# robflynnyh/long-context-asr

Measured on AMD Instinct MI355X. Metric: spectrogram-frames/sec (6L/768D, seq=16384), higher is better.
Workload: dtype bf16; 1 GPU; 6L/768D/6H SConformerXL, seq=16384, rotary theta=1.5M, fwd+CTC+bwd+clip+MADGRAD; per_gpu_batch=128, global_batch=128, seq_len=16384, parallelism=dp1

## Files before the change

### long-context-asr_amd/csrc/attention.hip

```cpp
#ifdef SCONF_ATTN_STAMP
#define SCONF_STAMPS
#endif
#include "common.h"
#include <algorithm>
#include <type_traits>
#include <vector>
#include <stdio.h>

namespace {

struct AttnParams {
    const bf16 *q, *k, *v;
    bf16* o;
    const bf16 *dout;
    bf16 *dq, *dk, *dv;
    float* lse;
    float* delta;
    long q_sb, q_sn, q_sh, k_sb, k_sn, k_sh, v_sb, v_sn, v_sh, o_sb, o_sn, o_sh;
    long do_sb, do_sn, do_sh, dq_sb, dq_sn, dq_sh, dk_sb, dk_sn, dk_sh, dv_sb, dv_sn, dv_sh;
    const int* lengths;
    int B, N, H;
    int win_left, win_right;
    float scale;
    const float *rot_cos, *rot_sin;
    unsigned long long* stamps;
};

#ifdef SCONF_ATTN_STAMP
#define STAMP_OUT(n) do { if (p.stamps && (threadIdx.x & 63) == 0) for (int i_ = 0; i_ < (n); ++i_) p.stamps[((long)blockIdx.x * 8 + (threadIdx.x >> 6)) * 8 + i_] = st_acc_[i_]; } while (0)
#else
#define STAMP_OUT(n)
#endif

struct BlkId { int b, h, x; };
__device__ __forceinline__ BlkId decode_block(const AttnParams& p, int nx) {
    const int total = nx * p.H * p.B, v = blockIdx.x;
    const int q = total >> 3, r = total & 7, xcd = v & 7;
    const int lid = (xcd < r ? xcd * (q + 1) : r * (q + 1) + (xcd - r) * q) + (v >> 3);
    BlkId o;
    o.x = lid % nx;
    const int bh = lid / nx;
    o.h = bh % p.H; o.b = bh / p.H;
    return o;
}

constexpr float RESCALE_LOG2 = 6.f;

template <int D> __device__ __forceinline__ int swz(int row) {
    if constexpr (D == 32) return (row >> 2) & 3;
    else if constexpr (D == 64) return (((row >> 1) & 1) << 2) | (((row >> 3) & 1) << 1) | ((row >> 2) & 1);
    else return ((row & 3) << 2) | ((row >> 2) & 3);
}
template <int D> __device__ __forceinline__ int tile_off(int row, int ch) {
    return row * (2 * D) + ((ch ^ swz<D>(row)) << 4);
// ... 42 lines not shown
}

template <int D> struct LaneOffs {
    int row[D / 16];
    int trlo[D / 32];
    __device__ __forceinline__ LaneOffs(int lane) {
#pragma unroll
        for (int st = 0; st < D / 16; ++st) row[st] = tile_off<D>(lane & 31, 2 * st + (lane >> 5));
        const int i = lane & 15, q4 = i >> 2, p4 = i & 3, G = (lane >> 4) & 1, hh = lane >> 5;
        const int row0 = 4 * hh + q4, sub = (p4 & 1) * 8;
#pragma unroll
        for (int db = 0; db < D / 32; ++db) trlo[db] = tile_off<D>(row0, db * 4 + 2 * G + (p4 >> 1)) + sub;
    }
};
template <int D> __device__ __forceinline__ bf16x8 frag_row(const char* s, const LaneOffs<D>& L, int rbase, int st) {
    return *reinterpret_cast<const bf16x8*>(s + rbase * 2 * D + L.row[st]);
}
template <int D> __device__ __forceinline__ bf16x8 frag_tr(const char* s, const LaneOffs<D>& L, int rb, int db, int x32 = 32) {
    bf16x4 lo = __builtin_amdgcn_ds_read_tr16_b64_v4bf16((lds_p4)(s + rb * 2 * D + L.trlo[db]));
    bf16x4 hi = __builtin_amdgcn_ds_read_tr16_b64_v4bf16((lds_p4)(s + rb * 2 * D + 16 * D + (L.trlo[db] ^ x32)));
    return __builtin_shufflevector(lo, hi, 0, 1, 2, 3, 4, 5, 6, 7);
}
template <int D> __device__ __forceinline__ void load_bfrags(bf16x8 (&f)[D / 16], const bf16* base, long sn, int row0, int nvalid, int lane) {
    const int r = row0 + (lane & 31);
#pragma unroll
    for (int st = 0; st < D / 16; ++st) {
        uint4 v = make_uint4(0, 0, 0, 0);
        if (r < nvalid) v = *reinterpret_cast<const uint4*>(base + (long)r * sn + 16 * st + 8 * (lane >> 5));
        f[st] = __builtin_bit_cast(bf16x8, v);
    }
}
template <int D> __device__ __forceinline__ float delta_from_frags(const bf16x8 (&gf)[D / 16], const bf16* op, long o_sn, int row0, int nvalid, int lane) {
    bf16x8 of[D / 16];
    load_bfrags<D>(of, op, o_sn, row0, nvalid, lane);
    float acc = 0.f;
#pragma unroll
    for (int st = 0; st < D / 16; ++st)
#pragma unroll
        for (int j = 0; j < 8; ++j) acc += (float)gf[st][j] * (float)of[st][j];
    return acc + __shfl_xor(acc, 32, 64);
}
__device__ __forceinline__ bf16x8 pack8(const f32x16& a, int s2) {
    bf16x8 p;
#pragma unroll
    for (int j = 0; j < 8; ++j) p[j] = (bf16)a[8 * s2 + j];
    return p;
}

template <int D> __device__ __forceinline__ void store_t(const f32x16 (&acc)[D / 32], bf16* dst_row, float sc, int hh) {
#pragma unroll
    for (int db = 0; db < D / 32; ++db)
#pragma unroll
        for (int r4 = 0; r4 < 4; ++r4) {
            float v[4];
#pragma unroll
            for (int e = 0; e < 4; ++e) v[e] = acc[db][4 * r4 + e] * sc;
            store4(dst_row + db * 32 + 8 * r4 + 4 * hh, v);
        }
}

template <int D> __device__ __forceinline__ void store_t_rot(f32x16 (&acc)[D / 32], bf16* dst_row, float sc, int hh, const float* cs, const float* sn) {
    if constexpr (D >= 64) {
#pragma unroll
        for (int db = 0; db < D / 64; ++db)
#pragma unroll
            for (int r4 = 0; r4 < 4; ++r4) {
                float c[4], s[4];
                load4(cs + db * 32 + 8 * r4 + 4 * hh, c); load4(sn + db * 32 + 8 * r4 + 4 * hh, s);
#pragma unroll
                for (int e = 0; e < 4; ++e) {
                    const float a = acc[db][4 * r4 + e], b = acc[db + D / 64][4 * r4 + e];
                    acc[db][4 * r4 + e] = a * c[e] + b * s[e];
                    acc[db + D / 64][4 * r4 + e] = b * c[e] - a * s[e];
                }
            }
    } else {
#pragma unroll
        for (int r4 = 0; r4 < 2; ++r4) {
            float c[4], s[4];
            load4(cs + 8 * r4 + 4 * hh, c); load4(sn + 8 * r4 + 4 * hh, s);
#pragma unroll
            for (int e = 0; e < 4; ++e) {
                const float a = acc[0][4 * r4 + e], b = acc[0][4 * r4 + 8 + e];
                acc[0][4 * r4 + e] = a * c[e] + b * s[e];
                acc[0][4 * r4 + 8 + e] = b * c[e] - a * s[e];
            }
        }
    }
    store_t<D>(acc, dst_row, sc, hh);
}

template <int D>
__global__ __launch_bounds__(256, D == 256 ? 1 : 2) void attn_fwd_kernel(const AttnParams p) {
    extern __shared__ __attribute__((aligned(16))) char smem[];
    constexpr int TB = 64 * 2 * D;
    const int tid = threadIdx.x, lane = tid & 63, wave = tid >> 6, hh = lane >> 5;
    const BlkId bid = decode_block(p, (p.N + 127) / 128);
    const int b = bid.b, h = bid.h, qb0 = bid.x * 128, q0 = qb0 + wave * 32;
    const int len = p.lengths ? p.lengths[b] : p.N;
    const bf16* qp = p.q + b * p.q_sb + h * p.q_sh;
    const bf16* kp = p.k + b * p.k_sb + h * p.k_sh;
    const bf16* vp = p.v + b * p.v_sb + h * p.v_sh;
    const int qi = q0 + (lane & 31);
    const float c = p.scale * 1.4426950408889634f;

    bf16x8 qf[D / 16];
    load_bfrags<D>(qf, qp, p.q_sn, q0, p.N, lane);
    const LaneOffs<D> L(lane);

    const int kv_lo = p.win_left < 0 ? 0 : max(0, qb0 - p.win_left);
    const int kv_hi = min(len, p.win_right < 0 ? len : qb0 + 128 + p.win_right);
// ... 94 lines not shown
                                         float& d0, float& d1, float& d2, float& d3) {
    asm("v_fma_f32 %0, %8, %12, %13\n\tv_fma_f32 %1, %9, %12, %14\n\tv_fma_f32 %2, %10, %12, %15\n\tv_fma_f32 %3, %11, %12, %16\n\t"
        "v_exp_f32 %0, %0\n\tv_exp_f32 %1, %1\n\tv_exp_f32 %2, %2\n\tv_exp_f32 %3, %3\n\t"
        "v_mul_f32 %4, %4, %0\n\tv_mul_f32 %5, %5, %1\n\tv_mul_f32 %6, %6, %2\n\tv_mul_f32 %7, %7, %3"
        : "=&v"(pr[0]), "=&v"(pr[1]), "=&v"(pr[2]), "=&v"(pr[3]), "+v"(d0), "+v"(d1), "+v"(d2), "+v"(d3)
        : "v"(s0), "v"(s1), "v"(s2), "v"(s3), "v"(c), "v"(n0), "v"(n1), "v"(n2), "v"(n3));
}
__device__ __forceinline__ void exp4_submul(float s0, float s1, float s2, float s3, float c, float nl, float nd, float& d0, float& d1, float& d2, float& d3) {
    float e0, e1, e2, e3;
    asm("v_fma_f32 %0, %8, %12, %13\n\tv_fma_f32 %1, %9, %12, %13\n\tv_fma_f32 %2, %10, %12, %13\n\tv_fma_f32 %3, %11, %12, %13\n\t"
        "v_exp_f32 %0, %0\n\tv_exp_f32 %1, %1\n\tv_exp_f32 %2, %2\n\tv_exp_f32 %3, %3\n\t"
        "v_add_f32 %4, %4, %14\n\tv_add_f32 %5, %5, %14\n\tv_add_f32 %6, %6, %14\n\tv_add_f32 %7, %7, %14\n\t"
        "v_mul_f32 %4, %4, %0\n\tv_mul_f32 %5, %5, %1\n\tv_mul_f32 %6, %6, %2\n\tv_mul_f32 %7, %7, %3"
        : "=&v"(e0), "=&v"(e1), "=&v"(e2), "=&v"(e3), "+v"(d0), "+v"(d1), "+v"(d2), "+v"(d3)
        : "v"(s0), "v"(s1), "v"(s2), "v"(s3), "v"(c), "v"(nl), "v"(nd));
}
__device__ __forceinline__ void mfma_guard(f32x16& a) { asm volatile("s_nop 15\n\ts_nop 3" : "+v"(a)); }
__device__ __forceinline__ void mfma_guard(f32x16& a, f32x16& b) { asm volatile("s_nop 15\n\ts_nop 3" : "+v"(a), "+v"(b)); }

template <int D>
__global__ __launch_bounds__(512) void attn_fwd8p_kernel(const AttnParams p) {
    constexpr int KT = 128;
    extern __shared__ __attribute__((aligned(16))) char smem[];
    constexpr int TB = KT * 2 * D;
    const int tid = threadIdx.x, lane = tid & 63, wave = tid >> 6, hh = lane >> 5;
    const BlkId bid = decode_block(p, (p.N + 255) / 256);
    const int b = bid.b, h = bid.h, qb0 = bid.x * 256, q0 = qb0 + wave * 32;
    const int len = p.lengths ? p.lengths[b] : p.N;
    const bf16* qp = p.q + b * p.q_sb + h * p.q_sh;
    const bf16* kp = p.k + b * p.k_sb + h * p.k_sh;
    const bf16* vp = p.v + b * p.v_sb + h * p.v_sh;
    const int qi = q0 + (lane & 31);
    const float c = p.scale * 1.4426950408889634f;

    bf16x8 qf[D / 16];
    load_bfrags<D>(qf, qp, p.q_sn, q0, p.N, lane);
    const LaneOffs<D> L(lane);

    const int kv_lo = p.win_left < 0 ? 0 : max(0, qb0 - p.win_left);
    const int kv_hi = min(len, p.win_right < 0 ? len : qb0 + 256 + p.win_right);
    const int t_lo = kv_lo / KT, t_hi = (kv_hi + KT - 1) / KT;
    const bool windowed = p.win_left >= 0 || p.win_right >= 0;

    const unsigned lds0 = __builtin_amdgcn_readfirstlane(lds_addr(smem));
    const int wave_u = __builtin_amdgcn_readfirstlane(wave);
    const srd_t ksrd = make_srd(kp, view_bytes<D>(p.N, p.k_sn)), vsrd = make_srd(vp, view_bytes<D>(p.N, p.v_sn));
// ... 29 lines not shown

    f32x16 o[D / 32];
#pragma unroll
    for (int i = 0; i < D / 32; ++i)
#pragma unroll
        for (int r = 0; r < 16; ++r) o[i][r] = 0.f;
    float mc = 0.f, l0 = 0.f, l1 = 0.f;
    if (t_lo < t_hi) issue(t_lo, 0);
    pin_frags(qf);
    wait_vm<0>();
    __syncthreads();
    if (t_lo < t_hi) {
        const int kv0 = t_lo * KT;
        f32x16 s0, s1;
        s_chain(smem, 0, s0); s_chain(smem, 1, s1);
        if (kv0 + 64 > kv_hi || windowed) { mask_block(s0, kv0); mask_block(s1, kv0 + 32); }
        float mx = -INFINITY;
#pragma unroll
        for (int r = 0; r < 16; ++r) mx = fmaxf(mx, fmaxf(s0[r], s1[r]));
        mx = fmaxf(mx, __shfl_xor(mx, 32, 64));
        mc = (mx > -INFINITY) ? mx * c : 0.f;
    }
    const float nmc = -mc;
    STAMP_DECL(8)
    auto exp_block = [&](f32x16& sb, bf16x8& plo, bf16x8& phi) {
        mfma_guard(sb);
#pragma unroll
        for (int g = 0; g < 4; ++g) {
            float e[4];
            exp4_sum(e, sb[4 * g], sb[4 * g + 1], sb[4 * g + 2], sb[4 * g + 3], c, nmc, l0, l1);
#pragma unroll
            for (int j = 0; j < 4; ++j) sb[4 * g + j] = e[j];
        }
        plo = pack8(sb, 0); phi = pack8(sb, 1);
    };
    auto half_tile = [&](const char* sKh, const char* sVh, int kv0, const bool MASKED) {
        f32x16 s0, s1;
        bf16x8 pf[2][2];
        s_chain(sKh, 0, s0);
        if (MASKED) mask_block(s0, kv0);
        STAMP(1);
        s_chain(sKh, 1, s1);
        exp_block(s0, pf[0][0], pf[0][1]);
        if (MASKED) mask_block(s1, kv0 + 32);
        STAMP(2);
#pragma unroll
        for (int i = 0; i < 8; ++i)
// ... 2 lines not shown
        STAMP(3);
#pragma unroll
        for (int i = 0; i < 8; ++i)
            o[i >> 1] = __builtin_amdgcn_mfma_f32_32x32x16_bf16(frag_tr<D>(sVh, L, 32 + 16 * (i & 1), i >> 1), pf[1][i & 1], o[i >> 1], 0, 0, 0);
        STAMP(4);
    };
    for (int t = t_lo; t < t_hi; ++t) {
        const int cur = (t - t_lo) & 1;
        const char* sK = smem + cur * 2 * TB;
        const char* sV = sK + TB;
        if (t + 1 < t_hi) issue(t + 1, cur ^ 1);
        STAMP(0);
        for (int half = 0; half < KT / 64; ++half) {
            const int kv0 = t * KT + half * 64;
            if (kv0 >= kv_hi) break;
            const char* sKh = sK + half * 64 * 2 * D;
            const char* sVh = sV + half * 64 * 2 * D;
            half_tile(sKh, sVh, kv0, kv0 + 64 > kv_hi || windowed);
        }
        wait_vm<0>();
        __syncthreads();
        STAMP(5);
    }
    STAMP_OUT(6);
    float l = l0 + l1;
    float lt = l + __shfl_xor(l, 32, 64);
    float mfin = mc;
    if (__syncthreads_or(qi < len && qi < p.N && !(lt > 0.f && lt < 1e37f))) {
#pragma unroll
        for (int i = 0; i < D / 32; ++i)
#pragma unroll
            for (int r = 0; r < 16; ++r) o[i][r] = 0.f;
        float m = -INFINITY;
        l = 0.f;
        if (t_lo < t_hi) issue(t_lo, 0);
        wait_vm<0>();
        __syncthreads();
        for (int t = t_lo; t < t_hi; ++t) {
            const int cur = (t - t_lo) & 1;
            const char* sK = smem + cur * 2 * TB;
            const char* sV = sK + TB;
            if (t + 1 < t_hi) issue(t + 1, cur ^ 1);
            for (int half = 0; half < KT / 64; ++half) {
                const int kv0 = t * KT + half * 64;
                if (kv0 >= kv_hi) break;
                const char* sKh = sK + half * 64 * 2 * D;
                const char* sVh = sV + half * 64 * 2 * D;
// ... 23 lines not shown
                }
                l += rs;
                const bf16x8 p00 = pack8(s0, 0), p01 = pack8(s0, 1), p10 = pack8(s1, 0), p11 = pack8(s1, 1);
#pragma unroll
                for (int db = 0; db < D / 32; ++db) {
                    o[db] = __builtin_amdgcn_mfma_f32_32x32x16_bf16(frag_tr<D>(sVh, L, 0, db), p00, o[db], 0, 0, 0);
                    o[db] = __builtin_amdgcn_mfma_f32_32x32x16_bf16(frag_tr<D>(sVh, L, 16, db), p01, o[db], 0, 0, 0);
                    o[db] = __builtin_amdgcn_mfma_f32_32x32x16_bf16(frag_tr<D>(sVh, L, 32, db), p10, o[db], 0, 0, 0);
                    o[db] = __builtin_amdgcn_mfma_f32_32x32x16_bf16(frag_tr<D>(sVh, L, 48, db), p11, o[db], 0, 0, 0);
                }
            }
            wait_vm<0>();
            __syncthreads();
        }
        lt = l + __shfl_xor(l, 32, 64);
        mfin = (m == -INFINITY) ? 0.f : m * c;
    }
    if (qi < p.N) {
        const bool live = qi < len && lt > 0.f;
        const float inv = live ? 1.f / lt : 0.f;
        store_t<D>(o, p.o + b * p.o_sb + (long)qi * p.o_sn + h * p.o_sh, inv, hh);
        if (hh == 0 && p.lse) p.lse[((long)b * p.H + h) * p.N + qi] = live ? (mfin + __log2f(lt)) * 0.6931471805599453f : INFINITY;
    }
}

template <int D>
__global__ __launch_bounds__(256, D == 256 ? 1 : 2) void attn_bwd_dkdv_kernel(const AttnParams p) {
    extern __shared__ __attribute__((aligned(16))) char smem[];
    constexpr int TB = 32 * 2 * D;
    constexpr int SB = 2 * TB + 256;
    const int tid = threadIdx.x, lane = tid & 63, wave = tid >> 6, hh = lane >> 5;
    const BlkId bid = decode_block(p, (p.N + 127) / 128);
    const int b = bid.b, h = bid.h, kb0 = bid.x * 128, k0 = kb0 + wave * 32;
    const int len = p.lengths ? p.lengths[b] : p.N;
    const bf16* qp = p.q + b * p.q_sb + h * p.q_sh;
    const bf16* kp = p.k + b * p.k_sb + h * p.k_sh;
    const bf16* vp = p.v + b * p.v_sb + h * p.v_sh;
    const bf16* gp = p.dout + b * p.do_sb + h * p.do_sh;
    const float* delp = p.delta + ((long)b * p.H + h) * p.N;
    const float* lsep = delp + (long)p.B * p.H * p.N;
    const int key = k0 + (lane & 31);
    const float c = p.scale * 1.4426950408889634f;

    bf16x8 kf[D / 16];
    load_bfrags<D>(kf, kp, p.k_sn, k0, p.N, lane);
    const LaneOffs<D> L(lane);
// ... 78 lines not shown
            }
        }
        const bf16x8 pb0 = pack8(s, 0), pb1 = pack8(s, 1), db0 = pack8(dp, 0), db1 = pack8(dp, 1);
#pragma unroll
        for (int db = 0; db < D / 32; ++db) {
            dvt[db] = __builtin_amdgcn_mfma_f32_32x32x16_bf16(frag_tr<D>(sG, L, 0, db), pb0, dvt[db], 0, 0, 0);
            dvt[db] = __builtin_amdgcn_mfma_f32_32x32x16_bf16(frag_tr<D>(sG, L, 16, db), pb1, dvt[db], 0, 0, 0);
            dkt[db] = __builtin_amdgcn_mfma_f32_32x32x16_bf16(frag_tr<D>(sQ, L, 0, db), db0, dkt[db], 0, 0, 0);
            dkt[db] = __builtin_amdgcn_mfma_f32_32x32x16_bf16(frag_tr<D>(sQ, L, 16, db), db1, dkt[db], 0, 0, 0);
        }
        if (t + 1 < t_hi) lstore_stats(smem + (cur ^ 1) * SB);
        __syncthreads();
    }
    if (key < p.N) {
        if (p.rot_cos) store_t_rot<D>(dkt, p.dk + b * p.dk_sb + (long)key * p.dk_sn + h * p.dk_sh, p.scale, lane >> 5, p.rot_cos + (long)key * (D / 2), p.rot_sin + (long)key * (D / 2));
        else store_t<D>(dkt, p.dk + b * p.dk_sb + (long)key * p.dk_sn + h * p.dk_sh, p.scale, lane >> 5);
        store_t<D>(dvt, p.dv + b * p.dv_sb + (long)key * p.dv_sn + h * p.dv_sh, 1.f, lane >> 5);
    }
}

template <int D>
__global__ __launch_bounds__(512) void attn_bwd_dkdv8_kernel(const AttnParams p) {
    extern __shared__ __attribute__((aligned(16))) char smem[];
    constexpr int QR = 64;
    constexpr int TB = QR * 2 * D;
    constexpr int SB = 2 * TB + 512;
    const int tid = threadIdx.x, lane = tid & 63, wave = tid >> 6, hh = lane >> 5;
    const BlkId bid = decode_block(p, (p.N + 255) / 256);
    const int b = bid.b, h = bid.h, kb0 = bid.x * 256, k0 = kb0 + wave * 32;
    const int len = p.lengths ? p.lengths[b] : p.N;
    const bf16* qp = p.q + b * p.q_sb + h * p.q_sh;
    const bf16* kp = p.k + b * p.k_sb + h * p.k_sh;
    const bf16* vp = p.v + b * p.v_sb + h * p.v_sh;
    const bf16* gp = p.dout + b * p.do_sb + h * p.do_sh;
    const float* delp = p.delta + ((long)b * p.H + h) * p.N;
    const float* lsep = delp + (long)p.B * p.H * p.N;
    const int key = k0 + (lane & 31);
    const float c = p.scale * 1.4426950408889634f;

    bf16x8 kf[D / 16];
    load_bfrags<D>(kf, kp, p.k_sn, k0, p.N, lane);
    const LaneOffs<D> L(lane);
    char* sVt = smem + 2 * SB;
    const unsigned lds0 = __builtin_amdgcn_readfirstlane(lds_addr(smem));
    dma_tile<D, 256, 512>(vp, p.v_sn, kb0, p.N, lds0 + (unsigned)(2 * SB), tid);
    const char* sVw = sVt + wave * 32 * 2 * D;
// ... 9 lines not shown

    f32x16 dkt[D / 32], dvt[D / 32];
#pragma unroll
    for (int i = 0; i < D / 32; ++i)
#pragma unroll
        for (int r = 0; r < 16; ++r) { dkt[i][r] = 0.f; dvt[i][r] = 0.f; }

    const srd_t qsrd = make_srd(qp, view_bytes<D>(p.N, p.q_sn)), gsrd = make_srd(gp, view_bytes<D>(p.N, p.do_sn));
    auto issue = [&](int t, int buf) {
        const int tid_ = opaque(tid);
        const unsigned qvoff = tile_voff<D, 512>(p.q_sn, tid_), gvoff = tile_voff<D, 512>(p.do_sn, tid_);
        const int wave_u = __builtin_amdgcn_readfirstlane(tid_ >> 6);
        dma_tile128<QR, true>(qsrd, qvoff, p.q_sn, t * QR, lds0 + (unsigned)(buf * SB), wave_u);
        dma_tile128<QR, true>(gsrd, gvoff, p.do_sn, t * QR, lds0 + (unsigned)(buf * SB + TB), wave_u);
        if (wave_u < 2) {
            const int q = min(t * QR + (tid_ & 63), p.N - 1);
            dma4_asm((wave_u == 0 ? lsep : delp) + q, lds0 + (unsigned)(buf * SB + 2 * TB) + 256u * (unsigned)wave_u);
        }
    };
    if (t_lo < t_hi) issue(t_lo, 0);
    pin_frags(kf);
    wait_vm<0>();
    __syncthreads();
    STAMP_DECL(8)
    for (int t = t_lo; t < t_hi; ++t) {
        const int cur = (t - t_lo) & 1;
        const char* sQ = smem + cur * SB;
        const char* sG = sQ + TB;
        const float* sL = reinterpret_cast<const float*>(sQ + 2 * TB);
        const float* sD = sL + 64;
        if (t + 1 < t_hi) issue(t + 1, cur ^ 1);
        const bool need_mask = mask_wg || (t + 1) * QR > len;
        const int x32 = opaque(32);
        const int hh = (opaque(tid) >> 5) & 1;
        STAMP(0);
#pragma unroll
        for (int sub = 0; sub < 2; ++sub) {
            const int rb = 32 * sub, q0 = t * QR + rb;
            f32x16 s, dp;
#pragma unroll
            for (int g = 0; g < 4; ++g) {
                const float4 d4 = *reinterpret_cast<const float4*>(sD + rb + 8 * g + 4 * hh);
                dp[4 * g] = d4.x; dp[4 * g + 1] = d4.y; dp[4 * g + 2] = d4.z; dp[4 * g + 3] = d4.w;
            }
#pragma unroll
            for (int r = 0; r < 16; ++r) s[r] = 0.f;
#pragma unroll
// ... 15 lines not shown
                exp4_mul(pr, s[4 * g], s[4 * g + 1], s[4 * g + 2], s[4 * g + 3], c, a.x, a.y, a.z, a.w, d0, d1, d2, d3);
                dp[4 * g] = d0; dp[4 * g + 1] = d1; dp[4 * g + 2] = d2; dp[4 * g + 3] = d3;
#pragma unroll
                for (int e = 0; e < 4; ++e) s[4 * g + e] = pr[e];
            }
            bf16x8 pb0 = pack8(s, 0), pb1 = pack8(s, 1), db0 = pack8(dp, 0), db1 = pack8(dp, 1);
#ifdef SCONF_ATTN_STAMP
            tie(pb0); tie(pb1); tie(db0); tie(db1);
#endif
            STAMP(2);
#pragma unroll
            for (int db = 0; db < D / 32; ++db) {
                dvt[db] = __builtin_amdgcn_mfma_f32_32x32x16_bf16(frag_tr<D>(sG, L, rb, db, x32), pb0, dvt[db], 0, 0, 0);
                dvt[db] = __builtin_amdgcn_mfma_f32_32x32x16_bf16(frag_tr<D>(sG, L, rb + 16, db, x32), pb1, dvt[db], 0, 0, 0);
                dkt[db] = __builtin_amdgcn_mfma_f32_32x32x16_bf16(frag_tr<D>(sQ, L, rb, db, x32), db0, dkt[db], 0, 0, 0);
                dkt[db] = __builtin_amdgcn_mfma_f32_32x32x16_bf16(frag_tr<D>(sQ, L, rb + 16, db, x32), db1, dkt[db], 0, 0, 0);
            }
            STAMP(3);
        }
        wait_vm<0>();
        __syncthreads();
        STAMP(4);
    }
    STAMP_OUT(5);
    if (key < p.N) {
        if (p.rot_cos) store_t_rot<D>(dkt, p.dk + b * p.dk_sb + (long)key * p.dk_sn + h * p.dk_sh, p.scale, lane >> 5, p.rot_cos + (long)key * (D / 2), p.rot_sin + (long)key * (D / 2));
        else store_t<D>(dkt, p.dk + b * p.dk_sb + (long)key * p.dk_sn + h * p.dk_sh, p.scale, lane >> 5);
        store_t<D>(dvt, p.dv + b * p.dv_sb + (long)key * p.dv_sn + h * p.dv_sh, 1.f, lane >> 5);
    }
}

template <int D>
__global__ __launch_bounds__(256, D == 256 ? 1 : 2) void attn_bwd_dq_kernel(const AttnParams p) {
    extern __shared__ __attribute__((aligned(16))) char smem[];
    constexpr int TB = 64 * 2 * D;
    const int tid = threadIdx.x, lane = tid & 63, wave = tid >> 6, hh = lane >> 5;
    const BlkId bid = decode_block(p, (p.N + 127) / 128);
    const int b = bid.b, h = bid.h, qb0 = bid.x * 128, q0 = qb0 + wave * 32;
    const int len = p.lengths ? p.lengths[b] : p.N;
    const bf16* qp = p.q + b * p.q_sb + h * p.q_sh;
    const bf16* kp = p.k + b * p.k_sb + h * p.k_sh;
    const bf16* vp = p.v + b * p.v_sb + h * p.v_sh;
    const bf16* gp = p.dout + b * p.do_sb + h * p.do_sh;
    const int qi = q0 + (lane & 31);
    const float c = p.scale * 1.4426950408889634f;
    const float lse2 = (qi < len) ? p.lse[((long)b * p.H + h) * p.N + qi] * 1.4426950408889634f : INFINITY;

    bf16x8 qf[D / 16], gf[D / 16];
    load_bfrags<D>(qf, qp, p.q_sn, q0, p.N, lane);
    load_bfrags<D>(gf, gp, p.do_sn, q0, p.N, lane);
    float dlt = delta_from_frags<D>(gf, p.o + b * p.o_sb + h * p.o_sh, p.o_sn, q0, p.N, lane);
    if (qi >= len) dlt = 0.f;
// ... 48 lines not shown
                    if (p.win_right >= 0) ok = ok && key <= qi + p.win_right;
                    dp[r] = ok ? __builtin_amdgcn_exp2f(s[r] * c - lse2) * (dp[r] - dlt) : 0.f;
                }
            }
            const bf16x8 d0 = pack8(dp, 0), d1 = pack8(dp, 1);
#pragma unroll
            for (int db = 0; db < D / 32; ++db) {
                dqt[db] = __builtin_amdgcn_mfma_f32_32x32x16_bf16(frag_tr<D>(sK, L, kt * 32, db), d0, dqt[db], 0, 0, 0);
                dqt[db] = __builtin_amdgcn_mfma_f32_32x32x16_bf16(frag_tr<D>(sK, L, kt * 32 + 16, db), d1, dqt[db], 0, 0, 0);
            }
        }
        __syncthreads();
    }
    if (qi < p.N) {
        if (p.rot_cos) store_t_rot<D>(dqt, p.dq + b * p.dq_sb + (long)qi * p.dq_sn + h * p.dq_sh, p.scale, hh, p.rot_cos + (long)qi * (D / 2), p.rot_sin + (long)qi * (D / 2));
        else store_t<D>(dqt, p.dq + b * p.dq_sb + (long)qi * p.dq_sn + h * p.dq_sh, p.scale, hh);
    }
}

template <int D>
__global__ __launch_bounds__(512) void attn_bwd_dq8_kernel(const AttnParams p) {
    constexpr int KT = 128;
    extern __shared__ __attribute__((aligned(16))) char smem[];
    constexpr int TB = KT * 2 * D;
    const int tid = threadIdx.x, lane = tid & 63, wave = tid >> 6, hh = lane >> 5;
    const BlkId bid = decode_block(p, (p.N + 255) / 256);
    const int b = bid.b, h = bid.h, qb0 = bid.x * 256, q0 = qb0 + wave * 32;
    const int len = p.lengths ? p.lengths[b] : p.N;
    const bf16* qp = p.q + b * p.q_sb + h * p.q_sh;
    const bf16* kp = p.k + b * p.k_sb + h * p.k_sh;
    const bf16* vp = p.v + b * p.v_sb + h * p.v_sh;
    const bf16* gp = p.dout + b * p.do_sb + h * p.do_sh;
    const int qi = q0 + (lane & 31);
    const float c = p.scale * 1.4426950408889634f;
    const float lse2 = (qi < len) ? p.lse[((long)b * p.H + h) * p.N + qi] * 1.4426950408889634f : INFINITY;

    bf16x8 qf[D / 16], gf[D / 16];
    load_bfrags<D>(qf, qp, p.q_sn, q0, p.N, lane);
    load_bfrags<D>(gf, gp, p.do_sn, q0, p.N, lane);
    float dlt = delta_from_frags<D>(gf, p.o + b * p.o_sb + h * p.o_sh, p.o_sn, q0, p.N, lane);
    if (qi >= len) dlt = 0.f;
    if (hh == 0 && qi < p.N) {
        const long si = ((long)b * p.H + h) * p.N + qi;
        p.delta[si] = -dlt;
        p.delta[(long)p.B * p.H * p.N + si] = -lse2;
    }
    const LaneOffs<D> L(lane);
    const bool windowed = p.win_left >= 0 || p.win_right >= 0;
    const int key_lo = p.win_left >= 0 ? max(0, qi - p.win_left) : 0;
    const int key_hi = p.win_right >= 0 ? min(len - 1, qi + p.win_right) : len - 1;
    const unsigned key_rng = key_hi >= key_lo ? (unsigned)(key_hi - key_lo) : 0u;
    const bool key_none = key_hi < key_lo;

    const int kv_lo = p.win_left < 0 ? 0 : max(0, qb0 - p.win_left);
    const int kv_hi = min(len, p.win_right < 0 ? len : qb0 + 256 + p.win_right);
    const int t_lo = kv_lo / KT, t_hi = (qb0 < len) ? (kv_hi + KT - 1) / KT : t_lo;

    f32x16 dqt[D / 32];
#pragma unroll
    for (int i = 0; i < D / 32; ++i)
#pragma unroll
        for (int r = 0; r < 16; ++r) dqt[i][r] = 0.f;

    const unsigned lds0 = __builtin_amdgcn_readfirstlane(lds_addr(smem));
    const int wave_u = __builtin_amdgcn_readfirstlane(wave);
    const srd_t ksrd = make_srd(kp, view_bytes<D>(p.N, p.k_sn)), vsrd = make_srd(vp, view_bytes<D>(p.N, p.v_sn));
    const unsigned kvoff = tile_voff<D, 512>(p.k_sn, tid), vvoff = tile_voff<D, 512>(p.v_sn, tid);
    auto issue = [&](int t, int buf) {
        dma_tile128<KT, true>(ksrd, kvoff, p.k_sn, t * KT, lds0 + (unsigned)(buf * 2 * TB), wave_u);
        dma_tile128<KT, true>(vsrd, vvoff, p.v_sn, t * KT, lds0 + (unsigned)(buf * 2 * TB + TB), wave_u);
    };
    if (t_lo < t_hi) issue(t_lo, 0);
    pin_frags(qf); pin_frags(gf);
    wait_vm<0>();
    __syncthreads();
    STAMP_DECL(8)
    for (int t = t_lo; t < t_hi; ++t) {
        const int cur = (t - t_lo) & 1;
        const char* sK = smem + cur * 2 * TB;
        const char* sV = sK + TB;
        if (t + 1 < t_hi) issue(t + 1, cur ^ 1);
        STAMP(0);
        const int kv0 = t * KT;
        const bool masked = windowed || kv0 + KT > kv_hi;
        const float nl = -lse2, nd = -dlt;
        f32x16 s2[2], dp2[2];
        auto chains = [&](int kt, f32x16& s, f32x16& dp) {
#pragma unroll
            for (int r = 0; r < 16; ++r) { s[r] = 0.f; dp[r] = 0.f; }
#pragma unroll
            for (int st = 0; st < D / 16; ++st) {
                s = __builtin_amdgcn_mfma_f32_32x32x16_bf16(frag_row<D>(sK, L, kt * 32, st), qf[st], s, 0, 0, 0);
                dp = __builtin_amdgcn_mfma_f32_32x32x16_bf16(frag_row<D>(sV, L, kt * 32, st), gf[st], dp, 0, 0, 0);
            }
        };
        chains(0, s2[0], dp2[0]);
        STAMP(1);
#pragma unroll
        for (int kt = 0; kt < KT / 32; ++kt) {
// ... 8 lines not shown
            mfma_guard(s, dp);
#pragma unroll
            for (int g = 0; g < 4; ++g) {
                float d0 = dp[4 * g], d1 = dp[4 * g + 1], d2 = dp[4 * g + 2], d3 = dp[4 * g + 3];
                exp4_submul(s[4 * g], s[4 * g + 1], s[4 * g + 2], s[4 * g + 3], c, nl, nd, d0, d1, d2, d3);
                dp[4 * g] = d0; dp[4 * g + 1] = d1; dp[4 * g + 2] = d2; dp[4 * g + 3] = d3;
            }
            bf16x8 d0 = pack8(dp, 0), d1 = pack8(dp, 1);
#ifdef SCONF_ATTN_STAMP
            tie(d0); tie(d1);
#endif
            STAMP(2);
#pragma unroll
            for (int db = 0; db < D / 32; ++db) {
                dqt[db] = __builtin_amdgcn_mfma_f32_32x32x16_bf16(frag_tr<D>(sK, L, kt * 32, db), d0, dqt[db], 0, 0, 0);
                dqt[db] = __builtin_amdgcn_mfma_f32_32x32x16_bf16(frag_tr<D>(sK, L, kt * 32 + 16, db), d1, dqt[db], 0, 0, 0);
            }
            STAMP(3);
        }
        wait_vm<0>();
        __syncthreads();
        STAMP(4);
    }
    STAMP_OUT(5);
    if (qi < p.N) {
        if (p.rot_cos) store_t_rot<D>(dqt, p.dq + b * p.dq_sb + (long)qi * p.dq_sn + h * p.dq_sh, p.scale, hh, p.rot_cos + (long)qi * (D / 2), p.rot_sin + (long)qi * (D / 2));
        else store_t<D>(dqt, p.dq + b * p.dq_sb + (long)qi * p.dq_sn + h * p.dq_sh, p.scale, hh);
    }
}

#ifdef SCONF_ATTN_STAMP
static unsigned long long* stamp_buf(long nwg, hipStream_t stream) {
    static unsigned long long* sbuf = nullptr; static long scap = 0;
    if (scap < nwg * 64) { if (sbuf) (void)hipFree(sbuf); (void)hipMalloc(&sbuf, nwg * 64 * 8); scap = nwg * 64; }
    (void)hipMemsetAsync(sbuf, 0, nwg * 64 * 8, stream);
    return sbuf;
}
static void stamp_report(const char* what, unsigned long long* sbuf, long nwg, double units_per_wave, int nseg, const char* const* nm, hipStream_t stream) {
    if (!getenv("SCONF_ATTN_STAMP_PRINT")) return;
    (void)hipStreamSynchronize(stream);
    std::vector<unsigned long long> hb(nwg * 64);
    (void)hipMemcpy(hb.data(), sbuf, nwg * 64 * 8, hipMemcpyDeviceToHost);
    double sums[2][8] = {};
    for (long w = 0; w < nwg * 8; ++w) for (int i = 0; i < 8; ++i) sums[(w & 7) >= 4][i] += (double)hb[w * 8 + i];
    const double n = (double)nwg * 4 * units_per_wave;
    for (int g = 0; g < 2; ++g) {
        double tot = 0; for (int i = 0; i < nseg; ++i) tot += sums[g][i];
        fprintf(stderr, "[%s stamps] waves %d-%d: cycles per unit %.0f:", what, 4 * g, 4 * g + 3, tot / n);
        for (int i = 0; i < nseg; ++i) fprintf(stderr, "  %s %.0f (%.1f%%)", nm[i], sums[g][i] / n, 100.0 * sums[g][i] / tot);
        fprintf(stderr, "\n");
    }
// ... 52 lines not shown
SCONF_API int sconf_attn_fwd(const void* q, const void* k, const void* v, void* o, float* lse, const int32_t* lengths,
                             int64_t B, int64_t N, int64_t H, int64_t D, const int64_t* q_strides, const int64_t* k_strides,
                             const int64_t* v_strides, const int64_t* o_strides, int win_left, int win_right, float scale,
                             hipStream_t stream) {
    int64_t all[12];
    for (int i = 0; i < 3; ++i) { all[i] = q_strides[i]; all[3 + i] = k_strides[i]; all[6 + i] = v_strides[i]; all[9 + i] = o_strides[i]; }
    if (check_common("sconf_attn_fwd", B, N, H, D, all, 12)) return 1;
    AttnParams p = {};
    p.q = (const bf16*)q; p.k = (const bf16*)k; p.v = (const bf16*)v; p.o = (bf16*)o; p.lse = lse; p.lengths = lengths;
    p.q_sb = q_strides[0]; p.q_sn = q_strides[1]; p.q_sh = q_strides[2];
    p.k_sb = k_strides[0]; p.k_sn = k_strides[1]; p.k_sh = k_strides[2];
    p.v_sb = v_strides[0]; p.v_sn = v_strides[1]; p.v_sh = v_strides[2];
    p.o_sb = o_strides[0]; p.o_sn = o_strides[1]; p.o_sh = o_strides[2];
    p.B = (int)B; p.N = (int)N; p.H = (int)H; p.win_left = win_left; p.win_right = win_right; p.scale = scale;
    set_lds_attrs();
    const dim3 grid((unsigned)(cdiv(N, 128) * H * B));
    if (use_wide(D, N, all, 3)) {
        const long nwg = cdiv(N, 256) * H * B;
#ifdef SCONF_ATTN_STAMP
        p.stamps = stamp_buf(nwg, stream);
#endif
        hipLaunchKernelGGL((attn_fwd8p_kernel<128>), dim3((unsigned)nwg), dim3(512), FWD8_LDS, stream, p);
#ifdef SCONF_ATTN_STAMP
        { static const char* nm[6] = {"dma-issue", "S0", "S1|exp0", "PV0|exp1", "PV1", "wait+barrier"}; stamp_report("fwd8 (unit = 64-key half-tile)", p.stamps, nwg, (double)((N + 63) / 64), 6, nm, stream); }
#endif
    } else if (D == 128) launch_fwd4<128>(p, grid, stream);
    else if (D == 256) launch_fwd4<256>(p, grid, stream);
    else if (D == 64) launch_fwd4<64>(p, grid, stream);
    else launch_fwd4<32>(p, grid, stream);
    SCONF_LAUNCH_OK("sconf_attn_fwd");
    return 0;
}

SCONF_API int sconf_attn_bwd(const void* q, const void* k, const void* v, const void* o, const void* dout, const float* lse,
                             float* delta, void* dq, void* dk, void* dv, const int32_t* lengths,
                             int64_t B, int64_t N, int64_t H, int64_t D, const int64_t* q_strides, const int64_t* k_strides,
                             const int64_t* v_strides, const int64_t* o_strides, const int64_t* do_strides,
                             const int64_t* dq_strides, const int64_t* dk_strides, const int64_t* dv_strides,
                             int win_left, int win_right, float scale, const float* rot_cos, const float* rot_sin, hipStream_t stream) {
    int64_t all[24];
    const int64_t* ss[8] = {q_strides, k_strides, v_strides, o_strides, do_strides, dq_strides, dk_strides, dv_strides};
    for (int j = 0; j < 8; ++j) for (int i = 0; i < 3; ++i) all[3 * j + i] = ss[j][i];
    if (check_common("sconf_attn_bwd", B, N, H, D, all, 24)) return 1;
    AttnParams p = {};
    p.q = (const bf16*)q; p.k = (const bf16*)k; p.v = (const bf16*)v; p.o = (bf16*)const_cast<void*>(o); p.dout = (const bf16*)dout;
    p.lse = const_cast<float*>(lse); p.delta = delta; p.dq = (bf16*)dq; p.dk = (bf16*)dk; p.dv = (bf16*)dv; p.lengths = lengths;
    p.q_sb = q_strides[0]; p.q_sn = q_strides[1]; p.q_sh = q_strides[2];
    p.k_sb = k_strides[0]; p.k_sn = k_strides[1]; p.k_sh = k_strides[2];
    p.v_sb = v_strides[0]; p.v_sn = v_strides[1]; p.v_sh = v_strides[2];
    p.o_sb = o_strides[0]; p.o_sn = o_strides[1]; p.o_sh = o_strides[2];
    p.do_sb = do_strides[0]; p.do_sn = do_strides[1]; p.do_sh = do_strides[2];
    p.dq_sb = dq_strides[0]; p.dq_sn = dq_strides[1]; p.dq_sh = dq_strides[2];
    p.dk_sb = dk_strides[0]; p.dk_sn = dk_strides[1]; p.dk_sh = dk_strides[2];
    p.dv_sb = dv_strides[0]; p.dv_sn = dv_strides[1]; p.dv_sh = dv_strides[2];
    p.B = (int)B; p.N = (int)N; p.H = (int)H; p.win_left = win_left; p.win_right = win_right; p.scale = scale;
    SCONF_REQUIRE((rot_cos == nullptr) == (rot_sin == nullptr), "sconf_attn_bwd: rot_cos and rot_sin go together");
    p.rot_cos = rot_cos; p.rot_sin = rot_sin;
    set_lds_attrs();
    const dim3 grid((unsigned)(cdiv(N, 128) * H * B));
    if (use_wide(D, N, all, 8)) {
        const long nwg = cdiv(N, 256) * H * B;
#ifdef SCONF_ATTN_STAMP
        p.stamps = stamp_buf(nwg, stream);
#endif
        hipLaunchKernelGGL((attn_bwd_dq8_kernel<128>), dim3((unsigned)nwg), dim3(512), FWD8_LDS, stream, p);
#ifdef SCONF_ATTN_STAMP
        { static const char* nm[5] = {"dma-issue", "S|dP chains", "exp*", "dQ chain", "wait+barrier"}; stamp_report("dq8 (unit = 32 keys)", p.stamps, nwg, (double)((N + 31) / 32), 5, nm, stream); }
        p.stamps = stamp_buf(nwg, stream);
#endif
        hipLaunchKernelGGL((attn_bwd_dkdv8_kernel<128>), dim3((unsigned)nwg), dim3(512), DKDV8_LDS, stream, p);
#ifdef SCONF_ATTN_STAMP
        { static const char* nm[5] = {"dma-issue", "S|dP chains", "exp*", "dV|dK chains", "wait+barrier"}; stamp_report("dkdv8 (unit = 32 queries)", p.stamps, nwg, (double)((N + 31) / 32), 5, nm, stream); }
#endif
    } else if (D == 128) launch_bwd4<128>(p, grid, stream);
    else if (D == 256) launch_bwd4<256>(p, grid, stream);
    else if (D == 64) launch_bwd4<64>(p, grid, stream);
    else launch_bwd4<32>(p, grid, stream);
    SCONF_LAUNCH_OK("sconf_attn_bwd");
    return 0;
}
```

### long-context-asr_amd/csrc/gfx950.h

```cpp
#pragma once

typedef const __attribute__((address_space(1))) void* gptr;
typedef __attribute__((address_space(3))) void* lptr;
typedef __attribute__((address_space(3))) bf16x4* lds_p4;
__device__ __forceinline__ unsigned lds_addr(const void* p) { return (unsigned)(size_t)(const __attribute__((address_space(3))) char*)p; }

template <int N> __device__ __forceinline__ void wait_vm() { asm volatile("s_waitcnt vmcnt(%0)" :: "n"(N) : "memory"); }
__device__ __forceinline__ void wait_lgkm0() { asm volatile("s_waitcnt lgkmcnt(0)" ::: "memory"); }
__device__ __forceinline__ void wait_lgkm0_barrier() { asm volatile("s_waitcnt lgkmcnt(0)\n\ts_barrier" ::: "memory"); }

template <typename T> __device__ __forceinline__ void tie(T& x) { asm volatile("" : "+v"(x)); }
__device__ __forceinline__ int opaque(int v) { tie(v); return v; }
__device__ __forceinline__ unsigned tie_s(unsigned x) { asm("" : "+s"(x)); return x; }
template <int NF> __device__ __forceinline__ void pin_frags(bf16x8 (&f)[NF]) {
#pragma unroll
    for (int i = 0; i < NF; ++i) tie(f[i]);
}

__device__ __forceinline__ int acc_row(int r, int hh) { return (r & 3) + 8 * (r >> 2) + 4 * hh; }

__device__ __forceinline__ void dma16_asm(const void* gsrc, unsigned lds_dst_wave_base) {
    unsigned keep;
    asm volatile("s_mov_b32 %0, m0\n\ts_mov_b32 m0, %2\n\ts_nop 0\n\tglobal_load_lds_dwordx4 %1, off\n\ts_mov_b32 m0, %0"
                 : "=&s"(keep) : "v"(gsrc), "s"(lds_dst_wave_base) : "memory");
}
__device__ __forceinline__ void dma4_asm(const void* gsrc, unsigned lds_dst_wave_base) {
    unsigned keep;
    asm volatile("s_mov_b32 %0, m0\n\ts_mov_b32 m0, %2\n\ts_nop 0\n\tglobal_load_lds_dword %1, off\n\ts_mov_b32 m0, %0"
                 : "=&s"(keep) : "v"(gsrc), "s"(lds_dst_wave_base) : "memory");
}

typedef __amdgpu_buffer_rsrc_t srd_t;
__device__ __forceinline__ srd_t make_srd(const void* base, long nbytes) {
    const unsigned long a = (unsigned long)base;
    const unsigned lo = __builtin_amdgcn_readfirstlane((unsigned)a), hi = __builtin_amdgcn_readfirstlane((unsigned)(a >> 32));
    const unsigned nb = __builtin_amdgcn_readfirstlane((unsigned)(nbytes > 0xffffffffL ? 0xffffffffL : nbytes));
    return __builtin_amdgcn_make_buffer_rsrc((void*)(((unsigned long)hi << 32) | lo), 0, nb, 0x00020000);
}
__device__ __forceinline__ srd_t make_srd_uniform(const void* base, long nbytes) {
    return __builtin_amdgcn_make_buffer_rsrc(const_cast<void*>(base), 0, (unsigned)(nbytes > 0xffffffffL ? 0xffffffffL : nbytes), 0x00020000);
}
__device__ __forceinline__ void dma_dword(srd_t srd, unsigned voff, unsigned soff, unsigned lds_base) {
// ... 35 lines not shown
```

Baseline: 7.075 million spectrogram-frames/sec.

## Widen attention epilogue stores, stage dK/dV through LDS, overlap dq8 prologue loads

The transposed-accumulator store now packs two 4-element groups into one 16-byte store, using permlane32 swaps to exchange halves between lanes. In the dK/dV kernel, results are staged in LDS and written out as coalesced full rows. In the dQ kernel, the Q/dO/O fragment loads use buffer loads and are issued together with the first K/V DMA, so the delta computation overlaps it. Rotary math is switched to FMAs, and timing stamps now also cover the prologue and epilogue phases. The cost is extra LDS traffic and a wait in the epilogue, plus reuse of the sVt LDS region as scratch after the main loop.

After: 7.114 million spectrogram-frames/sec, median of 6. About the same (+0.5%).

```diff
diff --git a/long-context-asr_amd/csrc/attention.hip b/long-context-asr_amd/csrc/attention.hip
--- a/long-context-asr_amd/csrc/attention.hip
+++ b/long-context-asr_amd/csrc/attention.hip
@@ -28,8 +28,10 @@
 
 #ifdef SCONF_ATTN_STAMP
 #define STAMP_OUT(n) do { if (p.stamps && (threadIdx.x & 63) == 0) for (int i_ = 0; i_ < (n); ++i_) p.stamps[((long)blockIdx.x * 8 + (threadIdx.x >> 6)) * 8 + i_] = st_acc_[i_]; } while (0)
+#define STAMP_DRAIN() wait_vm<0>()
 #else
 #define STAMP_OUT(n)
+#define STAMP_DRAIN()
 #endif
 
 struct BlkId { int b, h, x; };
@@ -118,23 +120,24 @@
     return __builtin_shufflevector(lo, hi, 0, 1, 2, 3, 4, 5, 6, 7);
 }
 template <int D> __device__ __forceinline__ void load_bfrags(bf16x8 (&f)[D / 16], const bf16* base, long sn, int row0, int nvalid, int lane) {
+    const srd_t srd = make_srd(base, view_bytes<D>(nvalid, sn));
     const int r = row0 + (lane & 31);
-#pragma unroll
-    for (int st = 0; st < D / 16; ++st) {
-        uint4 v = make_uint4(0, 0, 0, 0);
-        if (r < nvalid) v = *reinterpret_cast<const uint4*>(base + (long)r * sn + 16 * st + 8 * (lane >> 5));
-        f[st] = __builtin_bit_cast(bf16x8, v);
-    }
+    const unsigned off = r < nvalid ? (unsigned)(r * sn * 2) + 16u * (unsigned)(lane >> 5) : 0u - 2u * D;
+#pragma unroll
+    for (int st = 0; st < D / 16; ++st) f[st] = __builtin_bit_cast(bf16x8, __builtin_amdgcn_raw_buffer_load_b128(srd, off + 32 * st, 0, 0));
+}
+template <int D> __device__ __forceinline__ float delta_sum(const bf16x8 (&gf)[D / 16], const bf16x8 (&of)[D / 16]) {
+    float acc = 0.f;
+#pragma unroll
+    for (int st = 0; st < D / 16; ++st)
+#pragma unroll
+        for (int j = 0; j < 8; ++j) acc += (float)gf[st][j] * (float)of[st][j];
+    return acc + __shfl_xor(acc, 32, 64);
 }
 template <int D> __device__ __forceinline__ float delta_from_frags(const bf16x8 (&gf)[D / 16], const bf16* op, long o_sn, int row0, int nvalid, int lane) {
     bf16x8 of[D / 16];
     load_bfrags<D>(of, op, o_sn, row0, nvalid, lane);
-    float acc = 0.f;
-#pragma unroll
-    for (int st = 0; st < D / 16; ++st)
-#pragma unroll
-        for (int j = 0; j < 8; ++j) acc += (float)gf[st][j] * (float)of[st][j];
-    return acc + __shfl_xor(acc, 32, 64);
+    return delta_sum<D>(gf, of);
 }
 __device__ __forceinline__ bf16x8 pack8(const f32x16& a, int s2) {
     bf16x8 p;
@@ -143,19 +146,39 @@
     return p;
 }
 
+template <int D> __device__ __forceinline__ uint4 pack_pair(const f32x16 (&acc)[D / 32], int db, int r4, float sc) {
+    bf16x4 t0, t1;
+#pragma unroll
+    for (int e = 0; e < 4; ++e) { t0[e] = (bf16)(acc[db][4 * r4 + e] * sc); t1[e] = (bf16)(acc[db][4 * r4 + 4 + e] * sc); }
+    uint2 a = __builtin_bit_cast(uint2, t0), b = __builtin_bit_cast(uint2, t1);
+    swap_halves(a.x, b.x); swap_halves(a.y, b.y);
+    return make_uint4(a.x, a.y, b.x, b.y);
+}
 template <int D> __device__ __forceinline__ void store_t(const f32x16 (&acc)[D / 32], bf16* dst_row, float sc, int hh) {
 #pragma unroll
     for (int db = 0; db < D / 32; ++db)
 #pragma unroll
-        for (int r4 = 0; r4 < 4; ++r4) {
-            float v[4];
-#pragma unroll
-            for (int e = 0; e < 4; ++e) v[e] = acc[db][4 * r4 + e] * sc;
-            store4(dst_row + db * 32 + 8 * r4 + 4 * hh, v);
-        }
-}
-
-template <int D> __device__ __forceinline__ void store_t_rot(f32x16 (&acc)[D / 32], bf16* dst_row, float sc, int hh, const float* cs, const float* sn) {
+        for (int r4 = 0; r4 < 4; r4 += 2) *reinterpret_cast<uint4*>(dst_row + db * 32 + 8 * r4 + 8 * hh) = pack_pair<D>(acc, db, r4, sc);
+}
+template <int D> __device__ __forceinline__ void store_t_rows(const f32x16 (&acc)[D / 32], char* slice, bf16* dst, long sn, int row0, int nrows, float sc, int lane) {
+    static_assert(D == 128, "one 256-byte row per 16 lanes");
+    const int hh = lane >> 5, r = lane & 31;
+#pragma unroll
+    for (int db = 0; db < D / 32; ++db)
+#pragma unroll
+        for (int r4 = 0; r4 < 4; r4 += 2) *reinterpret_cast<uint4*>(slice + tile_off<D>(r, db * 4 + r4 + hh)) = pack_pair<D>(acc, db, r4, sc);
+    wait_lgkm0();
+#pragma unroll
+    for (int i = 0; i < 8; ++i) {
+        const int row = 4 * i + (lane >> 4);
+        const uint4 v = *reinterpret_cast<const uint4*>(slice + tile_off<D>(row, lane & 15));
+        if (row0 + row < nrows) *reinterpret_cast<uint4*>(dst + (long)row * sn + 8 * (lane & 15)) = v;
+    }
+}
+
+__device__ __forceinline__ float rot_lo(float a, float b, float c, float s) { return __builtin_fmaf(b, s, a * c); }
+__device__ __forceinline__ float rot_hi(float a, float b, float c, float s) { return __builtin_fmaf(b, c, -(a * s)); }
+template <int D> __device__ __forceinline__ void rot_t(f32x16 (&acc)[D / 32], int hh, const float* cs, const float* sn) {
     if constexpr (D >= 64) {
 #pragma unroll
         for (int db = 0; db < D / 64; ++db)
@@ -166,8 +189,8 @@
 #pragma unroll
                 for (int e = 0; e < 4; ++e) {
                     const float a = acc[db][4 * r4 + e], b = acc[db + D / 64][4 * r4 + e];
-                    acc[db][4 * r4 + e] = a * c[e] + b * s[e];
-                    acc[db + D / 64][4 * r4 + e] = b * c[e] - a * s[e];
+                    acc[db][4 * r4 + e] = rot_lo(a, b, c[e], s[e]);
+                    acc[db + D / 64][4 * r4 + e] = rot_hi(a, b, c[e], s[e]);
                 }
             }
     } else {
@@ -178,11 +201,14 @@
 #pragma unroll
             for (int e = 0; e < 4; ++e) {
                 const float a = acc[0][4 * r4 + e], b = acc[0][4 * r4 + 8 + e];
-                acc[0][4 * r4 + e] = a * c[e] + b * s[e];
-                acc[0][4 * r4 + 8 + e] = b * c[e] - a * s[e];
-            }
-        }
-    }
+                acc[0][4 * r4 + e] = rot_lo(a, b, c[e], s[e]);
+                acc[0][4 * r4 + 8 + e] = rot_hi(a, b, c[e], s[e]);
+            }
+        }
+    }
+}
+template <int D> __device__ __forceinline__ void store_t_rot(f32x16 (&acc)[D / 32], bf16* dst_row, float sc, int hh, const float* cs, const float* sn) {
+    rot_t<D>(acc, hh, cs, sn);
     store_t<D>(acc, dst_row, sc, hh);
 }
 
@@ -323,6 +349,7 @@
 __global__ __launch_bounds__(512) void attn_fwd8p_kernel(const AttnParams p) {
     constexpr int KT = 128;
     extern __shared__ __attribute__((aligned(16))) char smem[];
+    STAMP_DECL(8)
     constexpr int TB = KT * 2 * D;
     const int tid = threadIdx.x, lane = tid & 63, wave = tid >> 6, hh = lane >> 5;
     const BlkId bid = decode_block(p, (p.N + 255) / 256);
@@ -398,7 +425,7 @@
         mc = (mx > -INFINITY) ? mx * c : 0.f;
     }
     const float nmc = -mc;
-    STAMP_DECL(8)
+    STAMP(6);
     auto exp_block = [&](f32x16& sb, bf16x8& plo, bf16x8& phi) {
         mfma_guard(sb);
 #pragma unroll
@@ -447,7 +474,6 @@
         __syncthreads();
         STAMP(5);
     }
-    STAMP_OUT(6);
     float l = l0 + l1;
     float lt = l + __shfl_xor(l, 32, 64);
     float mfin = mc;
@@ -517,6 +543,8 @@
         store_t<D>(o, p.o + b * p.o_sb + (long)qi * p.o_sn + h * p.o_sh, inv, hh);
         if (hh == 0 && p.lse) p.lse[((long)b * p.H + h) * p.N + qi] = live ? (mfin + __log2f(lt)) * 0.6931471805599453f : INFINITY;
     }
+    STAMP_DRAIN(); STAMP(7);
+    STAMP_OUT(8);
 }
 
 template <int D>
@@ -641,6 +669,7 @@
 template <int D>
 __global__ __launch_bounds__(512) void attn_bwd_dkdv8_kernel(const AttnParams p) {
     extern __shared__ __attribute__((aligned(16))) char smem[];
+    STAMP_DECL(8)
     constexpr int QR = 64;
     constexpr int TB = QR * 2 * D;
     constexpr int SB = 2 * TB + 512;
@@ -696,7 +725,7 @@
     pin_frags(kf);
     wait_vm<0>();
     __syncthreads();
-    STAMP_DECL(8)
+    STAMP(5);
     for (int t = t_lo; t < t_hi; ++t) {
         const int cur = (t - t_lo) & 1;
         const char* sQ = smem + cur * SB;
@@ -758,12 +787,11 @@
         __syncthreads();
         STAMP(4);
     }
-    STAMP_OUT(5);
-    if (key < p.N) {
-        if (p.rot_cos) store_t_rot<D>(dkt, p.dk + b * p.dk_sb + (long)key * p.dk_sn + h * p.dk_sh, p.scale, lane >> 5, p.rot_cos + (long)key * (D / 2), p.rot_sin + (long)key * (D / 2));
-        else store_t<D>(dkt, p.dk + b * p.dk_sb + (long)key * p.dk_sn + h * p.dk_sh, p.scale, lane >> 5);
-        store_t<D>(dvt, p.dv + b * p.dv_sb + (long)key * p.dv_sn + h * p.dv_sh, 1.f, lane >> 5);
-    }
+    if (key < p.N && p.rot_cos) rot_t<D>(dkt, lane >> 5, p.rot_cos + (long)key * (D / 2), p.rot_sin + (long)key * (D / 2));
+    store_t_rows<D>(dkt, sVt + wave * 32 * 2 * D, p.dk + b * p.dk_sb + (long)k0 * p.dk_sn + h * p.dk_sh, p.dk_sn, k0, p.N, p.scale, lane);
+    store_t_rows<D>(dvt, sVt + wave * 32 * 2 * D, p.dv + b * p.dv_sb + (long)k0 * p.dv_sn + h * p.dv_sh, p.dv_sn, k0, p.N, 1.f, lane);
+    STAMP_DRAIN(); STAMP(6);
+    STAMP_OUT(7);
 }
 
 template <int D>
@@ -858,6 +886,7 @@
 __global__ __launch_bounds__(512) void attn_bwd_dq8_kernel(const AttnParams p) {
     constexpr int KT = 128;
     extern __shared__ __attribute__((aligned(16))) char smem[];
+    STAMP_DECL(8)
     constexpr int TB = KT * 2 * D;
     const int tid = threadIdx.x, lane = tid & 63, wave = tid >> 6, hh = lane >> 5;
     const BlkId bid = decode_block(p, (p.N + 255) / 256);
@@ -869,35 +898,13 @@
     const bf16* gp = p.dout + b * p.do_sb + h * p.do_sh;
     const int qi = q0 + (lane & 31);
     const float c = p.scale * 1.4426950408889634f;
-    const float lse2 = (qi < len) ? p.lse[((long)b * p.H + h) * p.N + qi] * 1.4426950408889634f : INFINITY;
-
-    bf16x8 qf[D / 16], gf[D / 16];
-    load_bfrags<D>(qf, qp, p.q_sn, q0, p.N, lane);
-    load_bfrags<D>(gf, gp, p.do_sn, q0, p.N, lane);
-    float dlt = delta_from_frags<D>(gf, p.o + b * p.o_sb + h * p.o_sh, p.o_sn, q0, p.N, lane);
-    if (qi >= len) dlt = 0.f;
-    if (hh == 0 && qi < p.N) {
-        const long si = ((long)b * p.H + h) * p.N + qi;
-        p.delta[si] = -dlt;
-        p.delta[(long)p.B * p.H * p.N + si] = -lse2;
-    }
-    const LaneOffs<D> L(lane);
-    const bool windowed = p.win_left >= 0 || p.win_right >= 0;
-    const int key_lo = p.win_left >= 0 ? max(0, qi - p.win_left) : 0;
-    const int key_hi = p.win_right >= 0 ? min(len - 1, qi + p.win_right) : len - 1;
-    const unsigned key_rng = key_hi >= key_lo ? (unsigned)(key_hi - key_lo) : 0u;
-    const bool key_none = key_hi < key_lo;
+    const srd_t lsrd = make_srd(p.lse + ((long)b * p.H + h) * p.N, (long)p.N * 4);
+    const float lse_q = __builtin_bit_cast(float, __builtin_amdgcn_raw_buffer_load_b32(lsrd, qi < len ? (unsigned)qi * 4u : 0xfffffffcu, 0, 0));
+    const float lse2 = (qi < len) ? lse_q * 1.4426950408889634f : INFINITY;
 
     const int kv_lo = p.win_left < 0 ? 0 : max(0, qb0 - p.win_left);
     const int kv_hi = min(len, p.win_right < 0 ? len : qb0 + 256 + p.win_right);
     const int t_lo = kv_lo / KT, t_hi = (qb0 < len) ? (kv_hi + KT - 1) / KT : t_lo;
-
-    f32x16 dqt[D / 32];
-#pragma unroll
-    for (int i = 0; i < D / 32; ++i)
-#pragma unroll
-        for (int r = 0; r < 16; ++r) dqt[i][r] = 0.f;
-
     const unsigned lds0 = __builtin_amdgcn_readfirstlane(lds_addr(smem));
     const int wave_u = __builtin_amdgcn_readfirstlane(wave);
     const srd_t ksrd = make_srd(kp, view_bytes<D>(p.N, p.k_sn)), vsrd = make_srd(vp, view_bytes<D>(p.N, p.v_sn));
@@ -906,11 +913,36 @@
         dma_tile128<KT, true>(ksrd, kvoff, p.k_sn, t * KT, lds0 + (unsigned)(buf * 2 * TB), wave_u);
         dma_tile128<KT, true>(vsrd, vvoff, p.v_sn, t * KT, lds0 + (unsigned)(buf * 2 * TB + TB), wave_u);
     };
+
+    bf16x8 qf[D / 16], gf[D / 16], of[D / 16];
+    load_bfrags<D>(qf, qp, p.q_sn, q0, p.N, lane);
+    load_bfrags<D>(gf, gp, p.do_sn, q0, p.N, lane);
+    load_bfrags<D>(of, p.o + b * p.o_sb + h * p.o_sh, p.o_sn, q0, p.N, lane);
     if (t_lo < t_hi) issue(t_lo, 0);
+    float dlt = delta_sum<D>(gf, of);
+    if (qi >= len) dlt = 0.f;
+    if (hh == 0 && qi < p.N) {
+        const long si = ((long)b * p.H + h) * p.N + qi;
+        p.delta[si] = -dlt;
+        p.delta[(long)p.B * p.H * p.N + si] = -lse2;
+    }
+    const LaneOffs<D> L(lane);
+    const bool windowed = p.win_left >= 0 || p.win_right >= 0;
+    const int key_lo = p.win_left >= 0 ? max(0, qi - p.win_left) : 0;
+    const int key_hi = p.win_right >= 0 ? min(len - 1, qi + p.win_right) : len - 1;
+    const unsigned key_rng = key_hi >= key_lo ? (unsigned)(key_hi - key_lo) : 0u;
+    const bool key_none = key_hi < key_lo;
+
+    f32x16 dqt[D / 32];
+#pragma unroll
+    for (int i = 0; i < D / 32; ++i)
+#pragma unroll
+        for (int r = 0; r < 16; ++r) dqt[i][r] = 0.f;
+
     pin_frags(qf); pin_frags(gf);
     wait_vm<0>();
     __syncthreads();
-    STAMP_DECL(8)
+    STAMP(5);
     for (int t = t_lo; t < t_hi; ++t) {
         const int cur = (t - t_lo) & 1;
         const char* sK = smem + cur * 2 * TB;
@@ -965,11 +997,12 @@
         __syncthreads();
         STAMP(4);
     }
-    STAMP_OUT(5);
     if (qi < p.N) {
         if (p.rot_cos) store_t_rot<D>(dqt, p.dq + b * p.dq_sb + (long)qi * p.dq_sn + h * p.dq_sh, p.scale, hh, p.rot_cos + (long)qi * (D / 2), p.rot_sin + (long)qi * (D / 2));
         else store_t<D>(dqt, p.dq + b * p.dq_sb + (long)qi * p.dq_sn + h * p.dq_sh, p.scale, hh);
     }
+    STAMP_DRAIN(); STAMP(6);
+    STAMP_OUT(7);
 }
 
 #ifdef SCONF_ATTN_STAMP
@@ -1068,7 +1101,7 @@
 #endif
         hipLaunchKernelGGL((attn_fwd8p_kernel<128>), dim3((unsigned)nwg), dim3(512), FWD8_LDS, stream, p);
 #ifdef SCONF_ATTN_STAMP
-        { static const char* nm[6] = {"dma-issue", "S0", "S1|exp0", "PV0|exp1", "PV1", "wait+barrier"}; stamp_report("fwd8 (unit = 64-key half-tile)", p.stamps, nwg, (double)((N + 63) / 64), 6, nm, stream); }
+        { static const char* nm[8] = {"dma-issue", "S0", "S1|exp0", "PV0|exp1", "PV1", "wait+barrier", "prologue", "epilogue"}; stamp_report("fwd8 (unit = 64-key half-tile)", p.stamps, nwg, (double)((N + 63) / 64), 8, nm, stream); }
 #endif
     } else if (D == 128) launch_fwd4<128>(p, grid, stream);
     else if (D == 256) launch_fwd4<256>(p, grid, stream);
@@ -1111,12 +1144,12 @@
 #endif
         hipLaunchKernelGGL((attn_bwd_dq8_kernel<128>), dim3((unsigned)nwg), dim3(512), FWD8_LDS, stream, p);
 #ifdef SCONF_ATTN_STAMP
-        { static const char* nm[5] = {"dma-issue", "S|dP chains", "exp*", "dQ chain", "wait+barrier"}; stamp_report("dq8 (unit = 32 keys)", p.stamps, nwg, (double)((N + 31) / 32), 5, nm, stream); }
+        { static const char* nm[7] = {"dma-issue", "S|dP chains", "exp*", "dQ chain", "wait+barrier", "prologue", "epilogue"}; stamp_report("dq8 (unit = 32 keys)", p.stamps, nwg, (double)((N + 31) / 32), 7, nm, stream); }
         p.stamps = stamp_buf(nwg, stream);
 #endif
         hipLaunchKernelGGL((attn_bwd_dkdv8_kernel<128>), dim3((unsigned)nwg), dim3(512), DKDV8_LDS, stream, p);
 #ifdef SCONF_ATTN_STAMP
-        { static const char* nm[5] = {"dma-issue", "S|dP chains", "exp*", "dV|dK chains", "wait+barrier"}; stamp_report("dkdv8 (unit = 32 queries)", p.stamps, nwg, (double)((N + 31) / 32), 5, nm, stream); }
+        { static const char* nm[7] = {"dma-issue", "S|dP chains", "exp*", "dV|dK chains", "wait+barrier", "prologue", "epilogue"}; stamp_report("dkdv8 (unit = 32 queries)", p.stamps, nwg, (double)((N + 31) / 32), 7, nm, stream); }
 #endif
     } else if (D == 128) launch_bwd4<128>(p, grid, stream);
     else if (D == 256) launch_bwd4<256>(p, grid, stream);
diff --git a/long-context-asr_amd/csrc/gfx950.h b/long-context-asr_amd/csrc/gfx950.h
--- a/long-context-asr_amd/csrc/gfx950.h
+++ b/long-context-asr_amd/csrc/gfx950.h
@@ -18,6 +18,11 @@
 }
 
 __device__ __forceinline__ int acc_row(int r, int hh) { return (r & 3) + 8 * (r >> 2) + 4 * hh; }
+
+__device__ __forceinline__ void swap_halves(unsigned& lo, unsigned& hi) {
+    const auto r = __builtin_amdgcn_permlane32_swap(lo, hi, false, false);
+    lo = r[0]; hi = r[1];
+}
 
 __device__ __forceinline__ void dma16_asm(const void* gsrc, unsigned lds_dst_wave_base) {
     unsigned keep;
```
